# GregVS/Racing-SLAM

Measured on AMD Instinct MI355X. Metric: match+triangulate+local-BA passes/sec @ 2k kpts/frame, 20-KF×10k-pt window, higher is better.
Workload: dtype u8 Hamming (match), f64 (DLT SVD, BA), f32 (gates)

## Files before the change

racing-slam_amd/csrc/ba_schur_body.h:

```cpp
#pragma once
#include "ba_common.h"
#include "ba_backsub_body.h"

#define IT_L 64
#define IT_L_SMALL 40
#define SCH_WAVES 8
#define SCH_SUBS 8
#define YT_STRIDE4 81
#define YT_STRIDE8 145
#define YT_DOUBLES (192 * YT_STRIDE4)
__host__ __device__ __forceinline__ int sch_tile_doubles(int it_l)
{
    const int a = 3 * it_l * YT_STRIDE4, b8 = 3 * (it_l / 2) * YT_STRIDE8;
    return ((a > b8 ? a : b8) + 1) & ~1;
}
#define SCH_PRE 3
#define SCH_MAXC_LDS 64

typedef __attribute__((ext_vector_type(4))) double d4;

__device__ __forceinline__ int rank_in_mask(uint64_t m0, uint64_t m1, int s)
{
    if (s < 64) return __popcll(m0 & ((1ull << s) - 1ull));
    return __popcll(m0) + __popcll(m1 & ((1ull << (s - 64)) - 1ull));
}

__device__ __forceinline__ int nth_set_bit(uint64_t m0, uint64_t m1, int r)
{
    uint64_t m = m0;
    int base = 0;
    const int c0 = __popcll(m0);
    if (r >= c0) { r -= c0; m = m1; base = 64; }
    for (int i = 0; i < r; i++) m &= m - 1;
    return base + __builtin_ctzll(m);
}

__device__ __forceinline__ bool chol3_inv(const double V[6], double Li[6], double I[6], double L[6])
{
    const double l00s = V[0];
    if (!(l00s > 0.0)) return false;
    const double i00 = rsqrt_nr(l00s);
    const double l10 = V[1] * i00, l20 = V[2] * i00;
    const double l11s = V[3] - l10 * l10;
    if (!(l11s > 0.0)) return false;
    const double i11 = rsqrt_nr(l11s);
    const double l21 = (V[4] - l20 * l10) * i11;
    const double l22s = V[5] - l20 * l20 - l21 * l21;
    if (!(l22s > 0.0)) return false;
    const double i22 = rsqrt_nr(l22s);
    const double i10 = -l10 * i00 * i11;
    const double i21 = -l21 * i11 * i22;
    const double i20 = -(l20 * i00 + l21 * i10) * i22;
    Li[0] = i00; Li[1] = i10; Li[2] = i11; Li[3] = i20; Li[4] = i21; Li[5] = i22;
    L[0] = l00s * i00; L[1] = l10; L[2] = l11s * i11; L[3] = l20; L[4] = l21; L[5] = l22s * i22;
    I[0] = i00 * i00 + i10 * i10 + i20 * i20;
    I[1] = i10 * i11 + i20 * i21;
    I[2] = i20 * i22;
    I[3] = i11 * i11 + i21 * i21;
    I[4] = i21 * i22;
    I[5] = i22 * i22;
    return isfinite(I[0]) && isfinite(I[3]) && isfinite(I[5]);
}

__device__ __forceinline__ void tile_rc(int t, int NT, int& r, int& c)
{
    r = 0;
    int rem = t, len = NT;
    while (rem >= len) { rem -= len; len--; r++; }
    c = r + rem;
}

template <int NM, int STRIDE>
__device__ __forceinline__ void syrk_tiles(const double* yt, int nchunks, const int* tr, const int* tc, d4* acc, int lr, int lk)
{
    double a0[NM], b0[NM], a1[NM], b1[NM];
    const double* col = yt + (size_t)lk * STRIDE + lr;
#pragma unroll
    for (int t = 0; t < NM; t++) { a0[t] = col[16 * tr[t]]; b0[t] = col[16 * tc[t]]; }
    for (int kc = 0; kc < nchunks; kc += 2) {
        const double* c1 = col + (size_t)(4 * min(kc + 1, nchunks - 1)) * STRIDE;
#pragma unroll
        for (int t = 0; t < NM; t++) { a1[t] = c1[16 * tr[t]]; b1[t] = c1[16 * tc[t]]; }
#pragma unroll
        for (int t = 0; t < NM; t++) acc[t] = __builtin_amdgcn_mfma_f64_16x16x4f64(a0[t], b0[t], acc[t], 0, 0, 0);
        const double* c2 = col + (size_t)(4 * min(kc + 2, nchunks - 1)) * STRIDE;
#pragma unroll
        for (int t = 0; t < NM; t++) { a0[t] = c2[16 * tr[t]]; b0[t] = c2[16 * tc[t]]; }
        if (kc + 1 < nchunks) {
#pragma unroll
            for (int t = 0; t < NM; t++) acc[t] = __builtin_amdgcn_mfma_f64_16x16x4f64(a1[t], b1[t], acc[t], 0, 0, 0);
        }
    }
}

template <int NT, int TPW, int STRIDE>
__device__ __forceinline__ void syrk_scatter(const double* yt, int nchunks, int ns, const int* gslot, int n,
                                             int wave, int nw, double* __restrict__ S, double* __restrict__ rhs)
{
    const int lane = threadIdx.x & 63;
    const int lr = lane & 15, lk = lane >> 4;
    const int nrow = 6 * ns;
    const int nt_used = (nrow + 16) / 16;
    const int ntiles = nt_used * (nt_used + 1) / 2;
    const int simd = wave & 3, pos = (simd + 3) & 3;
    const int nws = (nw - simd + 3) >> 2;
    d4 acc[TPW];
    int tr[TPW], tc[TPW];
    int nmine = 0;
#pragma unroll
    for (int t = 0; t < TPW; t++) {
        acc[t] = (d4){0.0, 0.0, 0.0, 0.0};
        tr[t] = 0; tc[t] = 0;
        const int tile = pos + 4 * ((wave >> 2) + nws * t);
        if (tile < ntiles) { tile_rc(tile, nt_used, tr[t], tc[t]); nmine = t + 1; }
    }
    static_assert(TPW >= 1 && TPW <= 3, "tiles per wave");
    switch (nmine) {
    case 1: syrk_tiles<1, STRIDE>(yt, nchunks, tr, tc, acc, lr, lk); break;
    case 2: if (TPW >= 2) syrk_tiles<(TPW >= 2 ? 2 : 1), STRIDE>(yt, nchunks, tr, tc, acc, lr, lk); break;
    case 3: if (TPW >= 3) syrk_tiles<(TPW >= 3 ? 3 : 1), STRIDE>(yt, nchunks, tr, tc, acc, lr, lk); break;
    default: break;
    }
#pragma unroll
    for (int t = 0; t < TPW; t++) {
        if (t >= nmine) continue;
#pragma unroll
        for (int reg = 0; reg < 4; reg++) {
            const int R = 16 * tr[t] + lk + 4 * reg, Cc = 16 * tc[t] + lr;
            const double v = acc[t][reg];
            if (R >= nrow || Cc > nrow || R > Cc) continue;
            const int gr = 6 * gslot[R / 6] + R % 6;
            if (Cc == nrow) atomicAdd(&rhs[gr], -v);
            else atomicAdd(&S[(size_t)gr * n + 6 * gslot[Cc / 6] + Cc % 6], -v);
        }
    }
}

template <int NM, int NS, bool PLAIN, int STRIDE>
__device__ __forceinline__ void syrk_tiles_sets(const double* yt, const double* Gt, int it_l, int nchunks, const int* tr, const int* tc,
                                                d4 (*acc)[3], int lr, int lk)
{
    constexpr int NG = PLAIN ? NS - 1 : NS;
    auto load = [&](int kc, double* a, double* bp, double (*yb)[3], double (*g)[3]) {
        const int col = 4 * kc + lk;
        const int p = col / 3, kk = col - 3 * p;
        const double* c0 = yt + (size_t)(3 * p) * STRIDE + lr;
        const double* ca = yt + (size_t)col * STRIDE + lr;
#pragma unroll
        for (int t = 0; t < NM; t++) {
            a[t] = ca[16 * tr[t]];
            if (PLAIN) bp[t] = ca[16 * tc[t]];
            yb[t][0] = c0[16 * tc[t]]; yb[t][1] = c0[STRIDE + 16 * tc[t]]; yb[t][2] = c0[2 * STRIDE + 16 * tc[t]];
        }
        const int i0 = kk, i1 = kk == 0 ? 1 : (kk == 1 ? 3 : 4), i2 = kk == 0 ? 2 : (kk == 1 ? 4 : 5);
#pragma unroll
        for (int s = 0; s < NG; s++) {
            const double* gp = Gt + ((size_t)s * it_l + p) * 6;
            g[s][0] = gp[i0]; g[s][1] = gp[i1]; g[s][2] = gp[i2];
        }
    };
    auto mma = [&](const double* a, const double* bp, const double (*yb)[3], const double (*g)[3]) {
#pragma unroll
        for (int t = 0; t < NM; t++) {
            if (PLAIN) acc[t][0] = __builtin_amdgcn_mfma_f64_16x16x4f64(a[t], bp[t], acc[t][0], 0, 0, 0);
#pragma unroll
            for (int s = 0; s < NG; s++) {
                const double bs = fma(yb[t][2], g[s][2], fma(yb[t][1], g[s][1], yb[t][0] * g[s][0]));
                acc[t][s + (PLAIN ? 1 : 0)] = __builtin_amdgcn_mfma_f64_16x16x4f64(a[t], bs, acc[t][s + (PLAIN ? 1 : 0)], 0, 0, 0);
            }
        }
    };
    double a0[NM], b0[NM], yb0[NM][3], g0[3][3], a1[NM], b1[NM], yb1[NM][3], g1[3][3];
    load(0, a0, b0, yb0, g0);
    for (int kc = 0; kc < nchunks; kc += 2) {
        load(min(kc + 1, nchunks - 1), a1, b1, yb1, g1);
        mma(a0, b0, yb0, g0);
        load(min(kc + 2, nchunks - 1), a0, b0, yb0, g0);
        if (kc + 1 < nchunks) mma(a1, b1, yb1, g1);
    }
}

template <int NS, bool PLAIN, int STRIDE>
__device__ __forceinline__ void syrk_scatter_sets(const double* yt, const double* Gt, int it_l, int nchunks, int ns, const int* gslot, int n,
                                                  int wave, int nw, double* __restrict__ S0, double* __restrict__ rhs0)
{
    const int lane = threadIdx.x & 63;
    const int lr = lane & 15, lk = lane >> 4;
    const int nrow = 6 * ns;
    const int nt_used = (nrow + 16) / 16;
    const int ntiles = nt_used * (nt_used + 1) / 2;
    const int simd = wave & 3, pos = (simd + 3) & 3;
    const int nws = (nw - simd + 3) >> 2;
    d4 acc[3][3];
    int tr[3], tc[3];
    int nmine = 0;
#pragma unroll
    for (int t = 0; t < 3; t++) {
#pragma unroll
        for (int s = 0; s < 3; s++) acc[t][s] = (d4){0.0, 0.0, 0.0, 0.0};
        tr[t] = 0; tc[t] = 0;
        const int tile = pos + 4 * ((wave >> 2) + nws * t);
        if (tile < ntiles) { tile_rc(tile, nt_used, tr[t], tc[t]); nmine = t + 1; }
    }
    switch (nmine) {
    case 1: syrk_tiles_sets<1, NS, PLAIN, STRIDE>(yt, Gt, it_l, nchunks, tr, tc, acc, lr, lk); break;
    case 2: syrk_tiles_sets<2, NS, PLAIN, STRIDE>(yt, Gt, it_l, nchunks, tr, tc, acc, lr, lk); break;
    case 3: syrk_tiles_sets<3, NS, PLAIN, STRIDE>(yt, Gt, it_l, nchunks, tr, tc, acc, lr, lk); break;
    default: break;
    }
    const size_t sS = (size_t)n * n;
#pragma unroll
    for (int t = 0; t < 3; t++) {
        if (t >= nmine) continue;
#pragma unroll
        for (int reg = 0; reg < 4; reg++) {
            const int R = 16 * tr[t] + lk + 4 * reg, Cc = 16 * tc[t] + lr;
            if (R >= nrow || Cc > nrow || R > Cc) continue;
            const int gr = 6 * gslot[R / 6] + R % 6;
            if (Cc == nrow) {
#pragma unroll
                for (int s = 0; s < NS; s++) atomicAdd(&rhs0[(size_t)s * n + gr], -acc[t][s][reg]);
            } else {
                double* dst = &S0[(size_t)gr * n + 6 * gslot[Cc / 6] + Cc % 6];
#pragma unroll
                for (int s = 0; s < NS; s++) atomicAdd(dst + s * sS, -acc[t][s][reg]);
            }
        }
    }
}

template <int NT, int TPW, int STRIDE>
__device__ __forceinline__ void syrk_scatter_plain(const double* yt, int nchunks, int ns, const int* gslot, int n,
                                             int wave, int nw, double* __restrict__ S, double* __restrict__ rhs)
{
    const int lane = threadIdx.x & 63;
    const int lr = lane & 15, lk = lane >> 4;
    const int nrow = 6 * ns;
    const int nt_used = (nrow + 16) / 16;
    d4 acc[TPW];
    int tr[TPW], tc[TPW];
#pragma unroll
    for (int t = 0; t < TPW; t++) {
        acc[t] = (d4){0.0, 0.0, 0.0, 0.0};
        int r = 0, c = NT;
        if (wave + nw * t < NT * (NT + 1) / 2) tile_rc(wave + nw * t, NT, r, c);
        tr[t] = r; tc[t] = c;
    }
#pragma unroll 4
    for (int kc = 0; kc < nchunks; kc++) {
        const double* col = yt + (size_t)(kc * 4 + lk) * STRIDE + lr;
#pragma unroll
        for (int t = 0; t < TPW; t++) {
            if (tc[t] < nt_used) {
                const double a = col[16 * tr[t]], bb = col[16 * tc[t]];
                acc[t] = __builtin_amdgcn_mfma_f64_16x16x4f64(a, bb, acc[t], 0, 0, 0);
            }
        }
    }
#pragma unroll
    for (int t = 0; t < TPW; t++) {
        if (tc[t] >= nt_used) continue;
#pragma unroll
        for (int reg = 0; reg < 4; reg++) {
            const int R = 16 * tr[t] + lk + 4 * reg, Cc = 16 * tc[t] + lr;
            const double v = acc[t][reg];
            if (R >= nrow || Cc > nrow || R > Cc) continue;
            const int gr = 6 * gslot[R / 6] + R % 6;
            if (Cc == nrow) atomicAdd(&rhs[gr], -v);
            else atomicAdd(&S[(size_t)gr * n + 6 * gslot[Cc / 6] + Cc % 6], -v);
        }
    }
}

#define SCH_UCAP 21
template <bool PREP_LDS, bool ROUND>
static __device__ __forceinline__ void ba_schur_body(const BaDims& d, const BaBufs& b, const BaOpt& opt, const BaGroup& g, int it,
                                                     const int item, BaState* st_sh)
{
    extern __shared__ __attribute__((aligned(16))) double lds[];
    BA_STAMP_DECL;
#if RS_STAMPS
    const unsigned long long t_item0 = wall_clock64();
#endif
    const int lane = threadIdx.x & 63;
    const int wave = __builtin_amdgcn_readfirstlane((int)(threadIdx.x >> 6));
    double* yt = lds;
    double* ulds = lds + sch_tile_doubles(g.it_l);
    double* cprep = ulds + SCH_UCAP * 42;
    int* gslot = (int*)(cprep + (PREP_LDS ? (size_t)d.C * BA_PREP_LDS : 0));
    const int nlds = SCH_UCAP * 42;
    const uint64_t um0 = g.item_mask[2 * (size_t)item], um1 = g.item_mask[2 * (size_t)item + 1];
    const int l = lane & 7, sub = lane >> 3;
    const int wl = 8 * wave + l;
    const int q = item * g.it_l + wl;
    const int4 lmq = (q < d.P && wl < g.it_l) ? g.lm[q] : make_int4(-1, 0, 0, 0);
    const int p = lmq.x, o0 = lmq.y, nobs = lmq.z;
    for (int i = threadIdx.x; i < nlds; i += blockDim.x) ulds[i] = 0.0;
    const int yt_used = max(3 * g.it_l * YT_STRIDE4, 3 * (g.it_l / 2) * YT_STRIDE8);
    for (int i = threadIdx.x; i < yt_used; i += blockDim.x) yt[i] = 0.0;
    const BaState st = ba_round_state(b, opt, it, st_sh, !ROUND && item == 0);
    if (st.done) return;
    const double* gprep = b.prep + (size_t)st.cur * d.C * BA_PREP;
    if (PREP_LDS)
        for (int i = threadIdx.x; i < d.C * BA_PREP; i += blockDim.x) cprep[(i / BA_PREP) * BA_PREP_LDS + i % BA_PREP] = gprep[i];
    const double* prep = PREP_LDS ? (const double*)cprep : gprep;
    constexpr int PSTR = PREP_LDS ? BA_PREP_LDS : BA_PREP;
    const double* Xp = b.Xp + (size_t)st.cur * d.P * 3;
    double X[3] = {0, 0, 0};
    if (p >= 0) { X[0] = Xp[3 * (size_t)p]; X[1] = Xp[3 * (size_t)p + 1]; X[2] = Xp[3 * (size_t)p + 2]; }
    int jj0 = sub + l; while (nobs > 0 && jj0 >= nobs) jj0 -= nobs;
    int cs0 = 0;
    float2 uv0 = make_float2(0.f, 0.f);
    if (sub < nobs) { cs0 = g.obs_cs[o0 + jj0]; uv0 = b.obs_uv[o0 + jj0]; }
    const int ns = __popcll(um0) + __popcll(um1);
    if (threadIdx.x < 24) gslot[threadIdx.x] = (int)threadIdx.x < ns ? nth_set_bit(um0, um1, threadIdx.x) : 0;
    __syncthreads();

    BA_STAMP(b, 0);
    const size_t rep_off = (size_t)(item & (BA_UREP - 1)) * b.cam_stride;
    double* rhs_rep = b.rhs + rep_off;
    double cost = 0.0, gmax = 0.0;
    double fail[BA_MAXSETS];
#pragma unroll
    for (int k = 0; k < BA_MAXSETS; k++) fail[k] = 0.0;
    double V[6] = {0, 0, 0, 0, 0, 0}, gv[3] = {0, 0, 0};
    ObsLin o;
    if (st.fresh)
    for (int j = sub; j < nobs; j += SCH_SUBS) {
        int cs = cs0;
        float2 uvv = uv0;
        if (j != sub) {
            int jj = j + l; while (jj >= nobs) jj -= nobs;
            cs = g.obs_cs[o0 + jj];
            uvv = b.obs_uv[o0 + jj];
        }
        const int c = cs & 0xFFFF;
        obs_eval<true>(prep + (size_t)c * PSTR, X, uvv, d, o);
        cost += 0.5 * o.rho;
        const double w = o.w;
        V[0] += w * (o.jp[0] * o.jp[0] + o.jp[3] * o.jp[3]);
        V[1] += w * (o.jp[0] * o.jp[1] + o.jp[3] * o.jp[4]);
        V[2] += w * (o.jp[0] * o.jp[2] + o.jp[3] * o.jp[5]);
        V[3] += w * (o.jp[1] * o.jp[1] + o.jp[4] * o.jp[4]);
        V[4] += w * (o.jp[1] * o.jp[2] + o.jp[4] * o.jp[5]);
        V[5] += w * (o.jp[2] * o.jp[2] + o.jp[5] * o.jp[5]);
#pragma unroll
        for (int k = 0; k < 3; k++) gv[k] += w * (o.jp[k] * o.r0 + o.jp[3 + k] * o.r1);
        const int s = (cs >> 16) - 1;
        if (s >= 0) {
            if (ns <= SCH_UCAP) {
                double* u = ulds + rank_in_mask(um0, um1, s) * 42;
#pragma unroll
                for (int a = 0; a < 6; a++) {
#pragma unroll
                    for (int e = a; e < 6; e++) atomicAdd(&u[a * 6 + e], w * (o.jc[a] * o.jc[e] + o.jc[6 + a] * o.jc[6 + e]));
                    atomicAdd(&u[36 + a], w * (o.jc[a] * o.r0 + o.jc[6 + a] * o.r1));
                }
            } else {
#pragma unroll
                for (int a = 0; a < 6; a++) {
#pragma unroll
                    for (int e = a; e < 6; e++) atomicAdd(&b.U[rep_off + s * 36 + a * 6 + e], w * (o.jc[a] * o.jc[e] + o.jc[6 + a] * o.jc[6 + e]));
                    atomicAdd(&b.gc[rep_off + 6 * s + a], w * (o.jc[a] * o.r0 + o.jc[6 + a] * o.r1));
                }
            }
        }
    }
    BA_STAMP(b, 1);
#pragma unroll
    for (int k = 0; k < 6; k++) { V[k] += __shfl_xor(V[k], 8, 64); V[k] += __shfl_xor(V[k], 16, 64); V[k] += __shfl_xor(V[k], 32, 64); }
#pragma unroll
    for (int k = 0; k < 3; k++) { gv[k] += __shfl_xor(gv[k], 8, 64); gv[k] += __shfl_xor(gv[k], 16, 64); gv[k] += __shfl_xor(gv[k], 32, 64); }
    if (p >= 0) {
        if (st.fresh) {
            if (sub == 0) {
#pragma unroll
                for (int k = 0; k < 6; k++) b.Vc[6 * (size_t)p + k] = V[k];
            }
        } else {
#pragma unroll
            for (int k = 0; k < 6; k++) V[k] = b.Vc[6 * (size_t)p + k];
#pragma unroll
            for (int k = 0; k < 3; k++) gv[k] = b.gp[3 * (size_t)p + k];
        }
    }

    double sp[3] = {1.0, 1.0, 1.0};
    const double Vd[3] = {V[0], V[3], V[5]};
    if (p >= 0) {
        if (sub == 0) gmax = fmax(fabs(gv[0]), fmax(fabs(gv[1]), fabs(gv[2])));
#pragma unroll
        for (int k = 0; k < 3; k++) {
            if (!st.have_scale) sp[k] = opt.jacobi ? 1.0 / (1.0 + sqrt(Vd[k])) : 1.0;
            else sp[k] = b.sp[3 * (size_t)p + k];
        }
        if (sub == 0) {
#pragma unroll
            for (int k = 0; k < 3; k++) {
                if (!st.have_scale) b.sp[3 * (size_t)p + k] = sp[k];
                b.gp[3 * (size_t)p + k] = gv[k];
            }
        }
    }
    __shared__ double redw[SCH_WAVES][2 + BA_MAXSETS];
    bool epilogue_done = false;
    auto epilogue = [&]() {
        epilogue_done = true;
        cost = wave_sum(cost);
#pragma unroll
        for (int k = 0; k < BA_MAXSETS; k++) fail[k] = wave_sum(fail[k]);
        gmax = wave_max_nonneg(gmax);
        const int nwaves = (int)(blockDim.x >> 6);
        if (lane == 0) {
            redw[wave][0] = cost; redw[wave][1] = gmax;
#pragma unroll
            for (int k = 0; k < BA_MAXSETS; k++) redw[wave][2 + k] = fail[k];
        }
        __syncthreads();
        if (threadIdx.x == 0) {
            double c = 0.0, gm = 0.0, f[BA_MAXSETS];
#pragma unroll
            for (int k = 0; k < BA_MAXSETS; k++) f[k] = 0.0;
            for (int w = 0; w < nwaves; w++) {
                c += redw[w][0]; gm = fmax(gm, redw[w][1]);
#pragma unroll
                for (int k = 0; k < BA_MAXSETS; k++) f[k] += redw[w][2 + k];
            }
            const size_t slot = (size_t)(item & (BA_NSLOT - 1)) * BA_SLOT_STRIDE;
            if (c != 0.0) atomicAdd(&b.scal[slot], c);
#pragma unroll
            for (int k = 0; k < BA_MAXSETS; k++)
                if (f[k] > 0.0) atomicAdd(&b.scal[slot + 1 + k], f[k]);
            if (gm > 0.0) atomic_max_nonneg(&b.gmax[slot], gm);
        }
        for (int i = threadIdx.x; i < min(ns, SCH_UCAP) * 42; i += blockDim.x) {
            const int s = gslot[i / 42], k = i % 42;
            const double v = ulds[i];
            if (v != 0.0) {
                if (k < 36) atomicAdd(&b.U[rep_off + s * 36 + k], v);
                else atomicAdd(&b.gc[rep_off + 6 * s + (k - 36)], v);
            }
        }
    };
    double Lprev[6] = {0, 0, 0, 0, 0, 0};
    bool prev_all_ok = false;
    double* Mt = (double*)(gslot + 32);
    int set_first = 0;
    if (st.nact > 1 && ns > 0 && ns <= 10) {
        double Li0[6] = {0, 0, 0, 0, 0, 0}, L0[6] = {0, 0, 0, 0, 0, 0};
        auto damped = [&](int set, double lam[3], double Li[6], double I[6], double Lc[6]) -> bool {
            const double radius = ba_set_radius(st, set);
#pragma unroll
            for (int k = 0; k < 3; k++) {
                const double s2 = sp[k] * sp[k];
                lam[k] = clampd(s2 * Vd[k], opt.dmin, opt.dmax) / (radius * s2);
            }
            const double Vdm[6] = {V[0] + lam[0], V[1], V[2], V[3] + lam[1], V[4], V[5] + lam[2]};
            const bool ok = chol3_inv(Vdm, Li, I, Lc);
            if (!ok) {
#pragma unroll
                for (int k = 0; k < 6; k++) { I[k] = 0.0; Li[k] = 0.0; Lc[k] = 0.0; }
            }
            return ok;
        };
        double lam0[3] = {0, 0, 0}, I0[6] = {0, 0, 0, 0, 0, 0};
        bool ok0 = false;
        if (p >= 0) ok0 = damped(0, lam0, Li0, I0, L0);
        if (__syncthreads_or((p >= 0 && !ok0) ? 1 : 0) == 0) {
#pragma unroll
            for (int set = 0; set < BA_MAXSETS; set++) {
                if (set >= st.nact) continue;
                double lam[3] = {lam0[0], lam0[1], lam0[2]}, Li[6], I[6] = {I0[0], I0[1], I0[2], I0[3], I0[4], I0[5]}, Lc[6];
                bool ok = ok0;
                if (set > 0 && p >= 0) ok = damped(set, lam, Li, I, Lc);
                if (set > 0 && p < 0) {
#pragma unroll
                    for (int k = 0; k < 6; k++) I[k] = 0.0;
                }
                if (p >= 0 && sub == 0) {
                    if (!ok) {
#pragma unroll
                        for (int k = 0; k < BA_MAXSETS; k++) fail[k] = (k == set) ? 1.0 : fail[k];
                    }
                    double* lamp_set = b.lamp + ((size_t)set * d.P + p) * 3;
                    double* vinv_set = b.Vinv + ((size_t)set * d.P + p) * 6;
#pragma unroll
                    for (int k = 0; k < 3; k++) lamp_set[k] = lam[k];
#pragma unroll
                    for (int k = 0; k < 6; k++) vinv_set[k] = I[k];
                }
                if (set > 0 && sub == 0 && wl < g.it_l) {
                    const double T00 = I[0] * L0[0] + I[1] * L0[1] + I[2] * L0[3], T01 = I[1] * L0[2] + I[2] * L0[4], T02 = I[2] * L0[5];
                    const double T10 = I[1] * L0[0] + I[3] * L0[1] + I[4] * L0[3], T11 = I[3] * L0[2] + I[4] * L0[4], T12 = I[4] * L0[5];
                    const double T20 = I[2] * L0[0] + I[4] * L0[1] + I[5] * L0[3], T21 = I[4] * L0[2] + I[5] * L0[4], T22 = I[5] * L0[5];
                    double* gt = Mt + ((size_t)(set - 1) * g.it_l + wl) * 6;
                    gt[0] = L0[0] * T00 + L0[1] * T10 + L0[3] * T20;
                    gt[1] = L0[0] * T01 + L0[1] * T11 + L0[3] * T21;
                    gt[2] = L0[0] * T02 + L0[1] * T12 + L0[3] * T22;
                    gt[3] = L0[2] * T11 + L0[4] * T21;
                    gt[4] = L0[2] * T12 + L0[4] * T22;
                    gt[5] = L0[5] * T22;
                }
            }
            const bool okall0 = ok0;
            const double t0 = Li0[0] * gv[0], t1 = Li0[1] * gv[0] + Li0[2] * gv[1], t2 = Li0[3] * gv[0] + Li0[4] * gv[1] + Li0[5] * gv[2];
            BA_STAMP(b, 2);
            if (p >= 0 && okall0 && wl < g.it_l) {
                for (int j = sub; j < nobs; j += SCH_SUBS) {
                    int cs = cs0;
                    float2 uvv = uv0;
                    if (j != sub) {
                        int jj = j + l; while (jj >= nobs) jj -= nobs;
                        cs = g.obs_cs[o0 + jj];
                        uvv = b.obs_uv[o0 + jj];
                    }
                    const int c = cs & 0xFFFF;
                    const int s = (cs >> 16) - 1;
                    if (s < 0) continue;
                    obs_eval<true>(prep + (size_t)c * PSTR, X, uvv, d, o);
                    const int pos = rank_in_mask(um0, um1, s);
                    double* dst = yt + (size_t)(3 * wl) * YT_STRIDE4 + 6 * pos;
#pragma unroll
                    for (int a = 0; a < 6; a++) {
                        const double w0 = o.w * (o.jc[a] * o.jp[0] + o.jc[6 + a] * o.jp[3]);
                        const double w1 = o.w * (o.jc[a] * o.jp[1] + o.jc[6 + a] * o.jp[4]);
                        const double w2 = o.w * (o.jc[a] * o.jp[2] + o.jc[6 + a] * o.jp[5]);
                        dst[a] = w0 * Li0[0];
                        dst[YT_STRIDE4 + a] = w0 * Li0[1] + w1 * Li0[2];
                        dst[2 * YT_STRIDE4 + a] = w0 * Li0[3] + w1 * Li0[4] + w2 * Li0[5];
                    }
                }
                if (sub == 0) {
                    double* dst = yt + (size_t)(3 * wl) * YT_STRIDE4 + 6 * ns;
                    dst[0] = t0; dst[YT_STRIDE4] = t1; dst[2 * YT_STRIDE4] = t2;
                }
            }
            __syncthreads();
            BA_STAMP(b, 4);
            epilogue();
            {
                const int nw = (int)(blockDim.x >> 6);
                double* const S0 = b.S + (size_t)((unsigned)item % (unsigned)b.srep) * b.s_rep_stride;
                const int nch = 3 * g.it_l / 4;
                if (st.nact == 2) syrk_scatter_sets<2, true, YT_STRIDE4>(yt, Mt, g.it_l, nch, ns, gslot, d.n, wave, nw, S0, rhs_rep);
                else syrk_scatter_sets<3, true, YT_STRIDE4>(yt, Mt, g.it_l, nch, ns, gslot, d.n, wave, nw, S0, rhs_rep);
                if (st.nact > 3) {
                    const double* Gt2 = Mt + (size_t)2 * g.it_l * 6;
                    double* const S3 = S0 + (size_t)3 * d.n * d.n;
                    double* const rhs3 = rhs_rep + (size_t)3 * d.n;
                    if (st.nact == 4) syrk_scatter_sets<1, false, YT_STRIDE4>(yt, Gt2, g.it_l, nch, ns, gslot, d.n, wave, nw, S3, rhs3);
                    else syrk_scatter_sets<2, false, YT_STRIDE4>(yt, Gt2, g.it_l, nch, ns, gslot, d.n, wave, nw, S3, rhs3);
                }
            }
            set_first = st.nact;
        }
    }
    for (int set = set_first; set < st.nact; set++) {
    const double radius = ba_set_radius(st, set);
    double* const S_set = b.S + (size_t)((unsigned)item % (unsigned)b.srep) * b.s_rep_stride + (size_t)set * d.n * d.n;
    double* const rhs_set = rhs_rep + (size_t)set * d.n;
    double Li[6] = {0, 0, 0, 0, 0, 0}, I[6] = {0, 0, 0, 0, 0, 0}, Lc[6] = {0, 0, 0, 0, 0, 0};
    bool ok = false;
    if (p >= 0) {
        double lam[3];
#pragma unroll
        for (int k = 0; k < 3; k++) {
            const double s2 = sp[k] * sp[k];
            lam[k] = clampd(s2 * Vd[k], opt.dmin, opt.dmax) / (radius * s2);
        }
        const double Vdm[6] = {V[0] + lam[0], V[1], V[2], V[3] + lam[1], V[4], V[5] + lam[2]};
        ok = chol3_inv(Vdm, Li, I, Lc);
        if (!ok) {
#pragma unroll
            for (int k = 0; k < 6; k++) { I[k] = 0.0; Li[k] = 0.0; Lc[k] = 0.0; }
            if (sub == 0) {
#pragma unroll
                for (int k = 0; k < BA_MAXSETS; k++) fail[k] = (k == set) ? 1.0 : fail[k];
            }
        }
        if (sub == 0) {
            double* lamp_set = b.lamp + ((size_t)set * d.P + p) * 3;
            double* vinv_set = b.Vinv + ((size_t)set * d.P + p) * 6;
#pragma unroll
            for (int k = 0; k < 3; k++) lamp_set[k] = lam[k];
#pragma unroll
            for (int k = 0; k < 6; k++) vinv_set[k] = I[k];
        }
    }
    const double t0 = Li[0] * gv[0], t1 = Li[1] * gv[0] + Li[2] * gv[1], t2 = Li[3] * gv[0] + Li[4] * gv[1] + Li[5] * gv[2];

    BA_STAMP(b, 2);
    if (ns > 0 && ns <= 21) {
        const bool big = ns > 10;
        const int nbatch = big ? 2 : 1, lb_n = big ? g.it_l / 2 : g.it_l;
        const int stride = big ? YT_STRIDE8 : YT_STRIDE4;
        const bool transform = !big && set > 0 && prev_all_ok;
        if (transform) {
            const int ncol = 3 * lb_n, nrow1 = 6 * ns + 1;
            if (p >= 0 && sub == 0) {
                double* mt = Mt + 6 * wl;
                mt[0] = Li[0] * Lprev[0];
                mt[1] = Li[1] * Lprev[0] + Li[2] * Lprev[1];
                mt[2] = Li[2] * Lprev[2];
                mt[3] = Li[3] * Lprev[0] + Li[4] * Lprev[1] + Li[5] * Lprev[3];
                mt[4] = Li[4] * Lprev[2] + Li[5] * Lprev[4];
                mt[5] = Li[5] * Lprev[5];
            }
            __syncthreads();
            for (int idx = threadIdx.x; idx < lb_n * nrow1; idx += blockDim.x) {
                const int lbq = idx / nrow1, r = idx - lbq * nrow1;
                if (item * g.it_l + lbq >= d.P) continue;
                double* c0 = yt + (size_t)(3 * lbq) * YT_STRIDE4 + r;
                const double* mt = Mt + 6 * lbq;
                const double y0 = c0[0], y1 = c0[YT_STRIDE4], y2 = c0[2 * YT_STRIDE4];
                c0[0] = y0 * mt[0];
                c0[YT_STRIDE4] = y0 * mt[1] + y1 * mt[2];
                c0[2 * YT_STRIDE4] = y0 * mt[3] + y1 * mt[4] + y2 * mt[5];
            }
            prev_all_ok = __syncthreads_or((p >= 0 && !ok) ? 1 : 0) == 0;
            const int nw = (int)(blockDim.x >> 6);
            syrk_scatter<4, 3, YT_STRIDE4>(yt, ncol / 4, ns, gslot, d.n, wave, nw, S_set, rhs_set);
        } else
        for (int bt = 0; bt < nbatch; bt++) {
            const int ncol = 3 * lb_n;
            if (bt > 0 || set > 0) {
                __syncthreads();
                for (int i = threadIdx.x; i < ncol * stride; i += blockDim.x) yt[i] = 0.0;
                __syncthreads();
            }
            BA_STAMP(b, 3);
            const int lb = wl - bt * lb_n;
            if (p >= 0 && ok && lb >= 0 && lb < lb_n) {
                for (int j = sub; j < nobs; j += SCH_SUBS) {
                    int cs = cs0;
                    float2 uvv = uv0;
                    if (j != sub) {
                        int jj = j + l; while (jj >= nobs) jj -= nobs;
                        cs = g.obs_cs[o0 + jj];
                        uvv = b.obs_uv[o0 + jj];
                    }
                    const int c = cs & 0xFFFF;
                    const int s = (cs >> 16) - 1;
                    if (s < 0) continue;
                    obs_eval<true>(prep + (size_t)c * PSTR, X, uvv, d, o);
                    const int pos = rank_in_mask(um0, um1, s);
                    double* dst = yt + (size_t)(3 * lb) * stride + 6 * pos;
#pragma unroll
                    for (int a = 0; a < 6; a++) {
                        const double w0 = o.w * (o.jc[a] * o.jp[0] + o.jc[6 + a] * o.jp[3]);
                        const double w1 = o.w * (o.jc[a] * o.jp[1] + o.jc[6 + a] * o.jp[4]);
                        const double w2 = o.w * (o.jc[a] * o.jp[2] + o.jc[6 + a] * o.jp[5]);
                        dst[a] = w0 * Li[0];
                        dst[stride + a] = w0 * Li[1] + w1 * Li[2];
                        dst[2 * stride + a] = w0 * Li[3] + w1 * Li[4] + w2 * Li[5];
                    }
                }
                if (sub == 0) {
                    double* dst = yt + (size_t)(3 * lb) * stride + 6 * ns;
                    dst[0] = t0; dst[stride] = t1; dst[2 * stride] = t2;
                }
            }
            prev_all_ok = __syncthreads_or((p >= 0 && !ok) ? 1 : 0) == 0;
            BA_STAMP(b, 4);
            const int nw = (int)(blockDim.x >> 6);
            if (big) {
                if (nw >= 8) syrk_scatter_plain<8, 5, YT_STRIDE8>(yt, ncol / 4, ns, gslot, d.n, wave, nw, S_set, rhs_set);
                else syrk_scatter_plain<8, 8, YT_STRIDE8>(yt, ncol / 4, ns, gslot, d.n, wave, nw, S_set, rhs_set);
            } else {
                syrk_scatter<4, 3, YT_STRIDE4>(yt, ncol / 4, ns, gslot, d.n, wave, nw, S_set, rhs_set);
            }
        }
    } else if (ns > 21) {
        if (p >= 0 && ok && sub == 0) {
            for (int oi = o0; oi < o0 + nobs; oi++) {
                const int si = b.slot[b.obs_cam[oi]];
                if (si < 0) continue;
                obs_eval<true>(prep + (size_t)b.obs_cam[oi] * PSTR, X, b.obs_uv[oi], d, o);
                double Y[18];
#pragma unroll
                for (int a = 0; a < 6; a++) {
                    const double w0 = o.w * (o.jc[a] * o.jp[0] + o.jc[6 + a] * o.jp[3]);
                    const double w1 = o.w * (o.jc[a] * o.jp[1] + o.jc[6 + a] * o.jp[4]);
                    const double w2 = o.w * (o.jc[a] * o.jp[2] + o.jc[6 + a] * o.jp[5]);
                    Y[a * 3 + 0] = w0 * I[0] + w1 * I[1] + w2 * I[2];
                    Y[a * 3 + 1] = w0 * I[1] + w1 * I[3] + w2 * I[4];
                    Y[a * 3 + 2] = w0 * I[2] + w1 * I[4] + w2 * I[5];
                    atomicAdd(&rhs_set[6 * si + a], -(Y[a * 3] * gv[0] + Y[a * 3 + 1] * gv[1] + Y[a * 3 + 2] * gv[2]));
                }
                ObsLin oj;
                for (int ojx = o0; ojx < o0 + nobs; ojx++) {
                    const int sj = b.slot[b.obs_cam[ojx]];
                    if (sj < si) continue;
                    obs_eval<true>(prep + (size_t)b.obs_cam[ojx] * PSTR, X, b.obs_uv[ojx], d, oj);
                    double* Sblk = S_set + (size_t)(6 * si) * d.n + 6 * sj;
#pragma unroll
                    for (int e = 0; e < 6; e++) {
                        const double w0 = oj.w * (oj.jc[e] * oj.jp[0] + oj.jc[6 + e] * oj.jp[3]);
                        const double w1 = oj.w * (oj.jc[e] * oj.jp[1] + oj.jc[6 + e] * oj.jp[4]);
                        const double w2 = oj.w * (oj.jc[e] * oj.jp[2] + oj.jc[6 + e] * oj.jp[5]);
#pragma unroll
                        for (int a = 0; a < 6; a++)
                            if (sj > si || a <= e)
                                atomicAdd(&Sblk[(size_t)a * d.n + e], -(Y[a * 3] * w0 + Y[a * 3 + 1] * w1 + Y[a * 3 + 2] * w2));
                    }
                }
            }
        }
    }
#pragma unroll
    for (int k = 0; k < 6; k++) Lprev[k] = Lc[k];
    }
    BA_STAMP(b, 5);
    if (!epilogue_done) epilogue();
    BA_STAMP(b, 6);
    BA_STAMP_FLUSH(b, 8);
    if (ROUND) {
#if RS_STAMPS
        if (threadIdx.x == 0) {
            const unsigned long long te = wall_clock64();
            atomicMax(b.dbg + 38, te);
            const unsigned long long key = ((te - t_item0) << 32) | ((unsigned long long)item << 8) | (unsigned long long)ns;
            atomicMax(b.dbg + 26, key);
            atomicMin(b.dbg + 27, key);
            atomicMax(b.dbg + 28, t_item0);
            atomicMin(b.dbg + 29, t_item0);
        }
#endif
        asm volatile("s_waitcnt vmcnt(0)" ::: "memory");
        __syncthreads();
#if RS_STAMPS
        if (threadIdx.x == 0) atomicMax(b.dbg + 37, wall_clock64());
#endif
        if (threadIdx.x == 0) __hip_atomic_fetch_add(b.dbg + BA_SDONE, 1ull, __ATOMIC_RELAXED, __HIP_MEMORY_SCOPE_AGENT);
    }
}
```

Measured before the change: 2124.

## Fuse all active sets into one SYRK pass and add k-loop timing stamps

The multi-set Schur SYRK path used to run up to two passes over the Y tiles (sets 0-2, then sets 3-4 with separate Gt). It now instantiates syrk_scatter_sets with NS up to 5, so each loaded A/Y fragment feeds every active set in one k-loop. A single-buffered, per-tile interleaved load schedule is used when NM*NS is large, to limit register pressure. Stamp hooks (a syncthreads only under RS_STAMPS) are also added. The change removes the repeated tile reads, at the cost of more accumulator registers, which may lower occupancy or cause spills.

Result: slower. 1957 (-7.8%).

```diff
diff --git a/racing-slam_amd/csrc/ba_schur_body.h b/racing-slam_amd/csrc/ba_schur_body.h
--- a/racing-slam_amd/csrc/ba_schur_body.h
+++ b/racing-slam_amd/csrc/ba_schur_body.h
@@ -93,9 +93,9 @@
     }
 }
 
-template <int NT, int TPW, int STRIDE>
+template <int NT, int TPW, int STRIDE, class Stamp>
 __device__ __forceinline__ void syrk_scatter(const double* yt, int nchunks, int ns, const int* gslot, int n,
-                                             int wave, int nw, double* __restrict__ S, double* __restrict__ rhs)
+                                             int wave, int nw, double* __restrict__ S, double* __restrict__ rhs, Stamp&& k_loop_done)
 {
     const int lane = threadIdx.x & 63;
     const int lr = lane & 15, lk = lane >> 4;
@@ -121,6 +121,7 @@
     case 3: if (TPW >= 3) syrk_tiles<(TPW >= 3 ? 3 : 1), STRIDE>(yt, nchunks, tr, tc, acc, lr, lk); break;
     default: break;
     }
+    k_loop_done();
 #pragma unroll
     for (int t = 0; t < TPW; t++) {
         if (t >= nmine) continue;
@@ -138,20 +139,23 @@
 
 template <int NM, int NS, bool PLAIN, int STRIDE>
 __device__ __forceinline__ void syrk_tiles_sets(const double* yt, const double* Gt, int it_l, int nchunks, const int* tr, const int* tc,
-                                                d4 (*acc)[3], int lr, int lk)
+                                                d4 (*acc)[NS], int lr, int lk)
 {
     constexpr int NG = PLAIN ? NS - 1 : NS;
+    auto load_tile = [&](int kc, int t, double* a, double* bp, double (*yb)[3]) {
+        const int col = 4 * kc + lk;
+        const int p = col / 3;
+        const double* c0 = yt + (size_t)(3 * p) * STRIDE + lr;
+        const double* ca = yt + (size_t)col * STRIDE + lr;
+        a[t] = ca[16 * tr[t]];
+        if (PLAIN) bp[t] = ca[16 * tc[t]];
+        yb[t][0] = c0[16 * tc[t]]; yb[t][1] = c0[STRIDE + 16 * tc[t]]; yb[t][2] = c0[2 * STRIDE + 16 * tc[t]];
+    };
     auto load = [&](int kc, double* a, double* bp, double (*yb)[3], double (*g)[3]) {
+#pragma unroll
+        for (int t = 0; t < NM; t++) load_tile(kc, t, a, bp, yb);
         const int col = 4 * kc + lk;
         const int p = col / 3, kk = col - 3 * p;
-        const double* c0 = yt + (size_t)(3 * p) * STRIDE + lr;
-        const double* ca = yt + (size_t)col * STRIDE + lr;
-#pragma unroll
-        for (int t = 0; t < NM; t++) {
-            a[t] = ca[16 * tr[t]];
-            if (PLAIN) bp[t] = ca[16 * tc[t]];
-            yb[t][0] = c0[16 * tc[t]]; yb[t][1] = c0[STRIDE + 16 * tc[t]]; yb[t][2] = c0[2 * STRIDE + 16 * tc[t]];
-        }
         const int i0 = kk, i1 = kk == 0 ? 1 : (kk == 1 ? 3 : 4), i2 = kk == 0 ? 2 : (kk == 1 ? 4 : 5);
 #pragma unroll
         for (int s = 0; s < NG; s++) {
@@ -159,30 +163,54 @@
             g[s][0] = gp[i0]; g[s][1] = gp[i1]; g[s][2] = gp[i2];
         }
     };
-    auto mma = [&](const double* a, const double* bp, const double (*yb)[3], const double (*g)[3]) {
-#pragma unroll
-        for (int t = 0; t < NM; t++) {
-            if (PLAIN) acc[t][0] = __builtin_amdgcn_mfma_f64_16x16x4f64(a[t], bp[t], acc[t][0], 0, 0, 0);
-#pragma unroll
-            for (int s = 0; s < NG; s++) {
-                const double bs = fma(yb[t][2], g[s][2], fma(yb[t][1], g[s][1], yb[t][0] * g[s][0]));
-                acc[t][s + (PLAIN ? 1 : 0)] = __builtin_amdgcn_mfma_f64_16x16x4f64(a[t], bs, acc[t][s + (PLAIN ? 1 : 0)], 0, 0, 0);
-            }
+    auto mma_tile = [&](int t, const double* a, const double* bp, const double (*yb)[3], const double (*g)[3]) {
+        if (PLAIN) acc[t][0] = __builtin_amdgcn_mfma_f64_16x16x4f64(a[t], bp[t], acc[t][0], 0, 0, 0);
+#pragma unroll
+        for (int s = 0; s < NG; s++) {
+            const double bs = fma(yb[t][2], g[s][2], fma(yb[t][1], g[s][1], yb[t][0] * g[s][0]));
+            acc[t][s + (PLAIN ? 1 : 0)] = __builtin_amdgcn_mfma_f64_16x16x4f64(a[t], bs, acc[t][s + (PLAIN ? 1 : 0)], 0, 0, 0);
         }
     };
-    double a0[NM], b0[NM], yb0[NM][3], g0[3][3], a1[NM], b1[NM], yb1[NM][3], g1[3][3];
-    load(0, a0, b0, yb0, g0);
-    for (int kc = 0; kc < nchunks; kc += 2) {
-        load(min(kc + 1, nchunks - 1), a1, b1, yb1, g1);
-        mma(a0, b0, yb0, g0);
-        load(min(kc + 2, nchunks - 1), a0, b0, yb0, g0);
-        if (kc + 1 < nchunks) mma(a1, b1, yb1, g1);
-    }
-}
-
-template <int NS, bool PLAIN, int STRIDE>
+    if constexpr (NM * NS <= 9) {
+        double a0[NM], b0[NM], yb0[NM][3], g0[NG][3], a1[NM], b1[NM], yb1[NM][3], g1[NG][3];
+        load(0, a0, b0, yb0, g0);
+        for (int kc = 0; kc < nchunks; kc += 2) {
+            load(min(kc + 1, nchunks - 1), a1, b1, yb1, g1);
+#pragma unroll
+            for (int t = 0; t < NM; t++) mma_tile(t, a0, b0, yb0, g0);
+            load(min(kc + 2, nchunks - 1), a0, b0, yb0, g0);
+            if (kc + 1 < nchunks) {
+#pragma unroll
+                for (int t = 0; t < NM; t++) mma_tile(t, a1, b1, yb1, g1);
+            }
+        }
+    } else {
+        double a0[NM], b0[NM], yb0[NM][3], g0[NG][3];
+        load(0, a0, b0, yb0, g0);
+        for (int kc = 0; kc < nchunks; kc++) {
+            const int kn = min(kc + 1, nchunks - 1);
+            double an[NM], bn[NM], ybn[NM][3];
+#pragma unroll
+            for (int t = 0; t < NM; t++) {
+                mma_tile(t, a0, b0, yb0, g0);
+                if (t + 1 < NM) load_tile(kn, t, an, bn, ybn);
+            }
+            double ah[NM], bh[NM], ybh[NM][3];
+            load(kn, ah, bh, ybh, g0);
+#pragma unroll
+            for (int t = 0; t < NM; t++) {
+                const bool last = t + 1 == NM;
+                a0[t] = last ? ah[t] : an[t];
+                if (PLAIN) b0[t] = last ? bh[t] : bn[t];
+                yb0[t][0] = last ? ybh[t][0] : ybn[t][0]; yb0[t][1] = last ? ybh[t][1] : ybn[t][1]; yb0[t][2] = last ? ybh[t][2] : ybn[t][2];
+            }
+        }
+    }
+}
+
+template <int NS, bool PLAIN, int STRIDE, class Stamp>
 __device__ __forceinline__ void syrk_scatter_sets(const double* yt, const double* Gt, int it_l, int nchunks, int ns, const int* gslot, int n,
-                                                  int wave, int nw, double* __restrict__ S0, double* __restrict__ rhs0)
+                                                  int wave, int nw, double* __restrict__ S0, double* __restrict__ rhs0, Stamp&& k_loop_done)
 {
     const int lane = threadIdx.x & 63;
     const int lr = lane & 15, lk = lane >> 4;
@@ -191,13 +219,13 @@
     const int ntiles = nt_used * (nt_used + 1) / 2;
     const int simd = wave & 3, pos = (simd + 3) & 3;
     const int nws = (nw - simd + 3) >> 2;
-    d4 acc[3][3];
+    d4 acc[3][NS];
     int tr[3], tc[3];
     int nmine = 0;
 #pragma unroll
     for (int t = 0; t < 3; t++) {
 #pragma unroll
-        for (int s = 0; s < 3; s++) acc[t][s] = (d4){0.0, 0.0, 0.0, 0.0};
+        for (int s = 0; s < NS; s++) acc[t][s] = (d4){0.0, 0.0, 0.0, 0.0};
         tr[t] = 0; tc[t] = 0;
         const int tile = pos + 4 * ((wave >> 2) + nws * t);
         if (tile < ntiles) { tile_rc(tile, nt_used, tr[t], tc[t]); nmine = t + 1; }
@@ -208,6 +236,7 @@
     case 3: syrk_tiles_sets<3, NS, PLAIN, STRIDE>(yt, Gt, it_l, nchunks, tr, tc, acc, lr, lk); break;
     default: break;
     }
+    k_loop_done();
     const size_t sS = (size_t)n * n;
 #pragma unroll
     for (int t = 0; t < 3; t++) {
@@ -442,6 +471,12 @@
             }
         }
     };
+    auto k_loop_done = [&]() {
+#if RS_STAMPS
+        __syncthreads();
+#endif
+        BA_STAMP(b, 7);
+    };
     double Lprev[6] = {0, 0, 0, 0, 0, 0};
     bool prev_all_ok = false;
     double* Mt = (double*)(gslot + 32);
@@ -542,14 +577,11 @@
                 const int nw = (int)(blockDim.x >> 6);
                 double* const S0 = b.S + (size_t)((unsigned)item % (unsigned)b.srep) * b.s_rep_stride;
                 const int nch = 3 * g.it_l / 4;
-                if (st.nact == 2) syrk_scatter_sets<2, true, YT_STRIDE4>(yt, Mt, g.it_l, nch, ns, gslot, d.n, wave, nw, S0, rhs_rep);
-                else syrk_scatter_sets<3, true, YT_STRIDE4>(yt, Mt, g.it_l, nch, ns, gslot, d.n, wave, nw, S0, rhs_rep);
-                if (st.nact > 3) {
-                    const double* Gt2 = Mt + (size_t)2 * g.it_l * 6;
-                    double* const S3 = S0 + (size_t)3 * d.n * d.n;
-                    double* const rhs3 = rhs_rep + (size_t)3 * d.n;
-                    if (st.nact == 4) syrk_scatter_sets<1, false, YT_STRIDE4>(yt, Gt2, g.it_l, nch, ns, gslot, d.n, wave, nw, S3, rhs3);
-                    else syrk_scatter_sets<2, false, YT_STRIDE4>(yt, Gt2, g.it_l, nch, ns, gslot, d.n, wave, nw, S3, rhs3);
+                switch (st.nact) {
+                case 2: syrk_scatter_sets<2, true, YT_STRIDE4>(yt, Mt, g.it_l, nch, ns, gslot, d.n, wave, nw, S0, rhs_rep, k_loop_done); break;
+                case 3: syrk_scatter_sets<3, true, YT_STRIDE4>(yt, Mt, g.it_l, nch, ns, gslot, d.n, wave, nw, S0, rhs_rep, k_loop_done); break;
+                case 4: syrk_scatter_sets<4, true, YT_STRIDE4>(yt, Mt, g.it_l, nch, ns, gslot, d.n, wave, nw, S0, rhs_rep, k_loop_done); break;
+                default: syrk_scatter_sets<5, true, YT_STRIDE4>(yt, Mt, g.it_l, nch, ns, gslot, d.n, wave, nw, S0, rhs_rep, k_loop_done); break;
                 }
             }
             set_first = st.nact;
@@ -619,7 +651,7 @@
             }
             prev_all_ok = __syncthreads_or((p >= 0 && !ok) ? 1 : 0) == 0;
             const int nw = (int)(blockDim.x >> 6);
-            syrk_scatter<4, 3, YT_STRIDE4>(yt, ncol / 4, ns, gslot, d.n, wave, nw, S_set, rhs_set);
+            syrk_scatter<4, 3, YT_STRIDE4>(yt, ncol / 4, ns, gslot, d.n, wave, nw, S_set, rhs_set, k_loop_done);
         } else
         for (int bt = 0; bt < nbatch; bt++) {
             const int ncol = 3 * lb_n;
@@ -667,7 +699,7 @@
                 if (nw >= 8) syrk_scatter_plain<8, 5, YT_STRIDE8>(yt, ncol / 4, ns, gslot, d.n, wave, nw, S_set, rhs_set);
                 else syrk_scatter_plain<8, 8, YT_STRIDE8>(yt, ncol / 4, ns, gslot, d.n, wave, nw, S_set, rhs_set);
             } else {
-                syrk_scatter<4, 3, YT_STRIDE4>(yt, ncol / 4, ns, gslot, d.n, wave, nw, S_set, rhs_set);
+                syrk_scatter<4, 3, YT_STRIDE4>(yt, ncol / 4, ns, gslot, d.n, wave, nw, S_set, rhs_set, k_loop_done);
             }
         }
     } else if (ns > 21) {
@@ -710,6 +742,10 @@
 #pragma unroll
     for (int k = 0; k < 6; k++) Lprev[k] = Lc[k];
     }
+#if RS_STAMPS
+    asm volatile("s_waitcnt vmcnt(0)" ::: "memory");
+    __syncthreads();
+#endif
     BA_STAMP(b, 5);
     if (!epilogue_done) epilogue();
     BA_STAMP(b, 6);
```
